# nyu-systems/Grendel-GS

Measured on NVIDIA H100. Metric: train-step Gaussians/s (preprocess+forward+loss+backward), higher is better.
Workload: dtype f32

## Files before the change

grendel-gs_b200/csrc/loss.cu:

```cuda
#include "common.cuh"

#define LS_TILE 32
#define LS_HALO 5
#define LS_IN (LS_TILE + 2 * LS_HALO)
#define LS_THREADS 256

__device__ __constant__ float c_gauss[11];
static unsigned long long g_gauss_ready = 0ull;

static int ensure_gauss() {
    int dev = 0;
    GS_CUDA_TRY(cudaGetDevice(&dev));
    if (dev < 64 && ((g_gauss_ready >> dev) & 1ull)) return GS_OK;
    float g[11], s = 0.f;
    for (int k = 0; k < 11; k++) { g[k] = (float)exp(-((double)(k - 5) * (k - 5)) / (2.0 * 1.5 * 1.5)); s += g[k]; }
    for (int k = 0; k < 11; k++) g[k] = g[k] / s;
    GS_CUDA_TRY(cudaMemcpyToSymbol(c_gauss, g, sizeof(g)));
    if (dev < 64) g_gauss_ready |= 1ull << dev;
    return GS_OK;
}

extern "C" size_t gs_loss_temp_bytes(int rows, int image_width) {
    return (size_t)9 * (size_t)(rows > 0 ? rows : 0) * (size_t)image_width * sizeof(float) + 256;
}

struct LossViews {
    int row0[GS_MAX_VIEWS], rows[GS_MAX_VIEWS];
    int crow0[GS_MAX_VIEWS], crow1[GS_MAX_VIEWS];
    const uint8_t *gt[GS_MAX_VIEWS];
    unsigned long long map_off[GS_MAX_VIEWS];
};

__global__ void __launch_bounds__(LS_THREADS)
k_loss_fwd(int W, int H, const LossViews lv, const float *__restrict__ image, float *__restrict__ maps,
           double *__restrict__ sums) {
    __shared__ float s_x[LS_IN][LS_IN + 1], s_y[LS_IN][LS_IN + 1];
    __shared__ float s_h[5][LS_IN][LS_TILE + 1];
    __shared__ float s_red[2][LS_THREADS / 32];
    const int view = blockIdx.z;
    const int row0 = lv.row0[view], rows = lv.rows[view], crow0 = lv.crow0[view], crow1 = lv.crow1[view];
    const int tx0 = blockIdx.x * LS_TILE, ty0 = blockIdx.y * LS_TILE;
    if (ty0 >= rows) return;
    const size_t HW = (size_t)H * W, SW = (size_t)rows * W;
    const uint8_t *__restrict__ gt = lv.gt[view];
    image += (size_t)view * 3 * HW;
    maps += lv.map_off[view];
    sums += 2 * view;
    const float C1 = 0.01f * 0.01f, C2 = 0.03f * 0.03f;
    float l1 = 0.f, ss = 0.f;
    for (int ch = 0; ch < 3; ch++) {
        for (int k = threadIdx.x; k < LS_IN * LS_IN; k += LS_THREADS) {
            const int r = k / LS_IN, c = k % LS_IN;
            const int y = ty0 + r - LS_HALO, x = tx0 + c - LS_HALO;
            float vx = 0.f, vy = 0.f;
            if (y >= 0 && y < rows && x >= 0 && x < W) {
                vx = image[ch * HW + (size_t)(row0 + y) * W + x];
                vy = fminf(1.f, fmaxf(0.f, (float)gt[ch * SW + (size_t)y * W + x] / 255.0f));
            }
            s_x[r][c] = vx; s_y[r][c] = vy;
        }
        __syncthreads();
        for (int k = threadIdx.x; k < LS_IN * (LS_TILE / 4); k += LS_THREADS) {
            const int r = k / (LS_TILE / 4), c0 = (k % (LS_TILE / 4)) * 4;
            float wx[14], wy[14];
#pragma unroll
            for (int t = 0; t < 14; t++) { wx[t] = s_x[r][c0 + t]; wy[t] = s_y[r][c0 + t]; }
#pragma unroll
            for (int q = 0; q < 4; q++) {
                float a0 = 0.f, a1 = 0.f, a2 = 0.f, a3 = 0.f, a4 = 0.f;
#pragma unroll
                for (int t = 0; t < 11; t++) {
                    const float g = c_gauss[t], vx = wx[q + t], vy = wy[q + t];
                    a0 += g * vx; a1 += g * vy; a2 += g * vx * vx; a3 += g * vy * vy; a4 += g * vx * vy;
                }
                s_h[0][r][c0 + q] = a0; s_h[1][r][c0 + q] = a1; s_h[2][r][c0 + q] = a2; s_h[3][r][c0 + q] = a3;
                s_h[4][r][c0 + q] = a4;
            }
        }
        __syncthreads();
        {
            const int c = threadIdx.x % LS_TILE, r0 = (threadIdx.x / LS_TILE) * 4, x = tx0 + c;
            float m1[4] = {0.f, 0.f, 0.f, 0.f}, m2[4] = {0.f, 0.f, 0.f, 0.f}, e11[4] = {0.f, 0.f, 0.f, 0.f},
                  e22[4] = {0.f, 0.f, 0.f, 0.f}, e12[4] = {0.f, 0.f, 0.f, 0.f};
#pragma unroll
            for (int t = 0; t < 14; t++) {
                const float v0 = s_h[0][r0 + t][c], v1 = s_h[1][r0 + t][c], v2 = s_h[2][r0 + t][c], v3 = s_h[3][r0 + t][c],
                            v4 = s_h[4][r0 + t][c];
#pragma unroll
                for (int q = 0; q < 4; q++) {
                    if (t - q >= 0 && t - q < 11) {
                        const float g = c_gauss[t - q];
                        m1[q] += g * v0; m2[q] += g * v1; e11[q] += g * v2; e22[q] += g * v3; e12[q] += g * v4;
                    }
                }
            }
#pragma unroll
            for (int q = 0; q < 4; q++) {
                const int r = r0 + q, y = ty0 + r;
                if (y < rows && x < W) {
                    const size_t o = (size_t)ch * SW + (size_t)y * W + x;
                    if (y < crow0 || y >= crow1) {
                        maps[o] = 0.f; maps[3 * SW + o] = 0.f; maps[6 * SW + o] = 0.f;
                    } else {
                        const float s1 = e11[q] - m1[q] * m1[q], s2 = e22[q] - m2[q] * m2[q], s12 = e12[q] - m1[q] * m2[q];
                        const float A = 2.f * m1[q] * m2[q] + C1, B = 2.f * s12 + C2,
                                    Cc = m1[q] * m1[q] + m2[q] * m2[q] + C1, D = s1 + s2 + C2;
                        const float iCD = 1.f / (Cc * D);
                        ss += A * B * iCD;
                        const float vx = s_x[r + LS_HALO][c + LS_HALO], vy = s_y[r + LS_HALO][c + LS_HALO];
                        l1 += fabsf(vx - vy);
                        maps[o] = 2.f * m2[q] * (B - A) * iCD - 2.f * m1[q] * A * B * (D - Cc) * iCD * iCD;
                        maps[3 * SW + o] = -A * B * iCD / D;
                        maps[6 * SW + o] = 2.f * A * iCD;
                    }
                }
            }
        }
        __syncthreads();
    }
#pragma unroll
    for (int o = 16; o > 0; o >>= 1) { l1 += __shfl_xor_sync(0xffffffffu, l1, o); ss += __shfl_xor_sync(0xffffffffu, ss, o); }
    if ((threadIdx.x & 31) == 0) { s_red[0][threadIdx.x >> 5] = l1; s_red[1][threadIdx.x >> 5] = ss; }
    __syncthreads();
    if (threadIdx.x == 0) {
        double a = 0.0, b = 0.0;
        for (int w = 0; w < LS_THREADS / 32; w++) { a += (double)s_red[0][w]; b += (double)s_red[1][w]; }
        atomicAdd(&sums[0], a); atomicAdd(&sums[1], b);
    }
}

__global__ void k_loss_finalize(int n, const double *__restrict__ sums, double inv_norm, float *__restrict__ out) {
    const int k = blockIdx.x * blockDim.x + threadIdx.x;
    if (k < 2 * n) out[k] = (float)(sums[k] * inv_norm);
}

__global__ void __launch_bounds__(LS_THREADS)
k_loss_bwd(int W, int H, const LossViews lv, const float *__restrict__ image, const float *__restrict__ maps,
           const float *__restrict__ grad_l1, const float *__restrict__ grad_ssim, float inv_norm,
           float *__restrict__ dimg) {
    __shared__ float s_m[3][LS_IN][LS_IN + 1];
    __shared__ float s_h[3][LS_IN][LS_TILE + 1];
    const int view = blockIdx.z;
    const int row0 = lv.row0[view], rows = lv.rows[view], crow0 = lv.crow0[view], crow1 = lv.crow1[view];
    const int tx0 = blockIdx.x * LS_TILE, ty0 = blockIdx.y * LS_TILE;
    if (ty0 >= rows) return;
    const size_t HW = (size_t)H * W, SW = (size_t)rows * W;
    const uint8_t *__restrict__ gt = lv.gt[view];
    image += (size_t)view * 3 * HW;
    dimg += (size_t)view * 3 * HW;
    maps += lv.map_off[view];
    const float gl1 = grad_l1[view] * inv_norm, gss = grad_ssim[view] * inv_norm;
    for (int ch = 0; ch < 3; ch++) {
        for (int k = threadIdx.x; k < LS_IN * LS_IN; k += LS_THREADS) {
            const int r = k / LS_IN, c = k % LS_IN;
            const int y = ty0 + r - LS_HALO, x = tx0 + c - LS_HALO;
            float v0 = 0.f, v1 = 0.f, v2 = 0.f;
            if (y >= 0 && y < rows && x >= 0 && x < W) {
                const size_t o = (size_t)ch * SW + (size_t)y * W + x;
                v0 = maps[o]; v1 = maps[3 * SW + o]; v2 = maps[6 * SW + o];
            }
            s_m[0][r][c] = v0; s_m[1][r][c] = v1; s_m[2][r][c] = v2;
        }
        __syncthreads();
        for (int k = threadIdx.x; k < LS_IN * (LS_TILE / 4); k += LS_THREADS) {
            const int r = k / (LS_TILE / 4), c0 = (k % (LS_TILE / 4)) * 4;
            float w0[14], w1[14], w2[14];
#pragma unroll
            for (int t = 0; t < 14; t++) { w0[t] = s_m[0][r][c0 + t]; w1[t] = s_m[1][r][c0 + t]; w2[t] = s_m[2][r][c0 + t]; }
#pragma unroll
            for (int q = 0; q < 4; q++) {
                float a0 = 0.f, a1 = 0.f, a2 = 0.f;
#pragma unroll
                for (int t = 0; t < 11; t++) {
                    const float g = c_gauss[t];
                    a0 += g * w0[q + t]; a1 += g * w1[q + t]; a2 += g * w2[q + t];
                }
                s_h[0][r][c0 + q] = a0; s_h[1][r][c0 + q] = a1; s_h[2][r][c0 + q] = a2;
            }
        }
        __syncthreads();
        {
            const int c = threadIdx.x % LS_TILE, r0 = (threadIdx.x / LS_TILE) * 4, x = tx0 + c;
            float b0[4] = {0.f, 0.f, 0.f, 0.f}, b1[4] = {0.f, 0.f, 0.f, 0.f}, b2[4] = {0.f, 0.f, 0.f, 0.f};
#pragma unroll
            for (int t = 0; t < 14; t++) {
                const float v0 = s_h[0][r0 + t][c], v1 = s_h[1][r0 + t][c], v2 = s_h[2][r0 + t][c];
#pragma unroll
                for (int q = 0; q < 4; q++) {
                    if (t - q >= 0 && t - q < 11) {
                        const float g = c_gauss[t - q];
                        b0[q] += g * v0; b1[q] += g * v1; b2[q] += g * v2;
                    }
                }
            }
#pragma unroll
            for (int q = 0; q < 4; q++) {
                const int y = ty0 + r0 + q;
                if (y < rows && x < W) {
                    const size_t oi = ch * HW + (size_t)(row0 + y) * W + x;
                    const float vx = image[oi];
                    const float vy = fminf(1.f, fmaxf(0.f, (float)gt[ch * SW + (size_t)y * W + x] / 255.0f));
                    const float d = vx - vy;
                    const float sgn = (y < crow0 || y >= crow1) ? 0.f : (d > 0.f ? 1.f : (d < 0.f ? -1.f : 0.f));
                    dimg[oi] = gl1 * sgn + gss * (b0[q] + 2.f * vx * b1[q] + vy * b2[q]);
                }
            }
        }
        __syncthreads();
    }
}

#define LS_HEADER_1 ((size_t)256)
#define LS_HEADER_B ((size_t)(2 * sizeof(double) * GS_MAX_VIEWS))

static int make_loss_views(int num_views, int H, int W, const int32_t *rows4, const void *const *gts, LossViews &lv,
                           int *max_rows, size_t *sum_rows) {
    GS_REQUIRE(num_views >= 1 && num_views <= GS_MAX_VIEWS, "num_views must be in [1, GS_MAX_VIEWS]");
    GS_REQUIRE(H > 0 && W > 0 && rows4 && gts, "sizes");
    size_t off = 0;
    int mx = 0;
    for (int v = 0; v < GS_MAX_VIEWS; v++) {
        lv.row0[v] = lv.rows[v] = lv.crow0[v] = lv.crow1[v] = 0;
        lv.gt[v] = nullptr;
        lv.map_off[v] = 0ull;
        if (v >= num_views) continue;
        const int row0 = rows4[4 * v], row1 = rows4[4 * v + 1], c0 = rows4[4 * v + 2], c1 = rows4[4 * v + 3];
        const int rows = row1 - row0;
        GS_REQUIRE(row0 >= 0 && row1 <= H && rows >= 0, "strip rows");
        if (rows == 0) continue;
        GS_REQUIRE(c0 >= row0 && c1 <= row1 && c1 >= c0, "count rows must lie inside [row0,row1)");
        GS_REQUIRE(gts[v] != nullptr, "null ground-truth pointer");
        lv.row0[v] = row0; lv.rows[v] = rows; lv.crow0[v] = c0 - row0; lv.crow1[v] = c1 - row0;
        lv.gt[v] = (const uint8_t *)gts[v];
        lv.map_off[v] = (unsigned long long)off;
        off += (size_t)9 * rows * W;
        mx = rows > mx ? rows : mx;
    }
    *max_rows = mx;
    *sum_rows = off / ((size_t)9 * W);
    return GS_OK;
}

static int loss_forward_impl(int num_views, int H, int W, const int32_t *rows4, const float *image, const void *const *gts,
                             float *out, void *temp, size_t temp_bytes, size_t header, cudaStream_t stream) {
    GS_REQUIRE(image && out && temp, "null pointer");
    LossViews lv;
    int max_rows = 0;
    size_t sum_rows = 0;
    int rc = make_loss_views(num_views, H, W, rows4, gts, lv, &max_rows, &sum_rows);
    if (rc != GS_OK) return rc;
    if (temp_bytes < header + (size_t)9 * sum_rows * W * sizeof(float)) {
        gs_set_error("gs_loss_forward: temp too small");
        return GS_ENOMEM;
    }
    rc = ensure_gauss();
    if (rc != GS_OK) return rc;
    double *sums = (double *)temp;
    float *maps = (float *)((char *)temp + header);
    GS_CUDA_TRY(cudaMemsetAsync(sums, 0, 2 * sizeof(double) * (size_t)num_views, stream));
    GsStageTimer timer(GS_STAGE_LOSS_FWD, stream);
    if (max_rows > 0) {
        dim3 grid((W + LS_TILE - 1) / LS_TILE, (max_rows + LS_TILE - 1) / LS_TILE, num_views);
        k_loss_fwd<<<grid, LS_THREADS, 0, stream>>>(W, H, lv, image, maps, sums);
        GS_LAUNCH_CHECK();
    }
    k_loss_finalize<<<1, 2 * GS_MAX_VIEWS, 0, stream>>>(num_views, sums, 1.0 / (3.0 * (double)H * (double)W), out);
    GS_LAUNCH_CHECK();
    return GS_OK;
}

static int loss_backward_impl(int num_views, int H, int W, const int32_t *rows4, const float *image,
                              const void *const *gts, const void *temp, const float *grad_l1, const float *grad_ssim,
                              float *dimg, size_t header, cudaStream_t stream) {
    GS_REQUIRE(image && temp && grad_l1 && grad_ssim && dimg, "null pointer");
    LossViews lv;
    int max_rows = 0;
    size_t sum_rows = 0;
    int rc = make_loss_views(num_views, H, W, rows4, gts, lv, &max_rows, &sum_rows);
    if (rc != GS_OK) return rc;
    rc = ensure_gauss();
    if (rc != GS_OK) return rc;
    const float *maps = (const float *)((const char *)temp + header);
    const size_t HW = (size_t)H * W;
    if (num_views == 1) {
        const int row0 = lv.row0[0], row1 = lv.row0[0] + lv.rows[0];
        for (int ch = 0; ch < 3; ch++) {
            if (row0 > 0) GS_CUDA_TRY(cudaMemsetAsync(dimg + ch * HW, 0, sizeof(float) * (size_t)row0 * W, stream));
            if (row1 < H)
                GS_CUDA_TRY(cudaMemsetAsync(dimg + ch * HW + (size_t)row1 * W, 0, sizeof(float) * (size_t)(H - row1) * W, stream));
        }
    } else if (sum_rows < (size_t)num_views * H) {
        GS_CUDA_TRY(cudaMemsetAsync(dimg, 0, sizeof(float) * 3 * HW * (size_t)num_views, stream));
    }
    if (max_rows == 0) return GS_OK;
    dim3 grid((W + LS_TILE - 1) / LS_TILE, (max_rows + LS_TILE - 1) / LS_TILE, num_views);
    GsStageTimer timer(GS_STAGE_LOSS_BWD, stream);
    k_loss_bwd<<<grid, LS_THREADS, 0, stream>>>(W, H, lv, image, maps, grad_l1, grad_ssim,
                                                (float)(1.0 / (3.0 * (double)H * (double)W)), dimg);
    GS_LAUNCH_CHECK();
    return GS_OK;
}

extern "C" int gs_loss_forward(int image_height, int image_width, int row0, int row1, int count_row0, int count_row1,
                               const float *image, const uint8_t *gt_u8, float *out_l1_ssim, void *temp,
                               size_t temp_bytes, void *stream_) {
    GS_REQUIRE(row1 > row0, "strip rows");
    GS_REQUIRE(gt_u8, "null pointer");
    const int32_t rows4[4] = {row0, row1, count_row0, count_row1};
    const void *gts[1] = {gt_u8};
    return loss_forward_impl(1, image_height, image_width, rows4, image, gts, out_l1_ssim, temp, temp_bytes, LS_HEADER_1,
                             (cudaStream_t)stream_);
}

extern "C" size_t gs_loss_temp_bytes_batched(int num_views, const int32_t *rows4_host, int image_width) {
    size_t rows = 0;
    for (int v = 0; v < num_views && rows4_host; v++) {
        const int r = rows4_host[4 * v + 1] - rows4_host[4 * v];
        rows += r > 0 ? (size_t)r : 0;
    }
    return LS_HEADER_B + (size_t)9 * rows * (size_t)(image_width > 0 ? image_width : 0) * sizeof(float) + 256;
}

extern "C" int gs_loss_forward_batched(int num_views, int image_height, int image_width, const int32_t *rows4_host,
                                       const float *image, const void *const *gt_u8_ptrs_host, float *out_l1_ssim,
                                       void *temp, size_t temp_bytes, void *stream_) {
    return loss_forward_impl(num_views, image_height, image_width, rows4_host, image, gt_u8_ptrs_host, out_l1_ssim, temp,
                             temp_bytes, LS_HEADER_B, (cudaStream_t)stream_);
}

extern "C" int gs_loss_backward(int image_height, int image_width, int row0, int row1, int count_row0, int count_row1,
                                const float *image, const uint8_t *gt_u8, const void *temp, const float *grad_l1,
                                const float *grad_ssim, float *dL_dimage, void *stream_) {
    GS_REQUIRE(row1 > row0, "strip rows");
    GS_REQUIRE(gt_u8, "null pointer");
    const int32_t rows4[4] = {row0, row1, count_row0, count_row1};
    const void *gts[1] = {gt_u8};
    return loss_backward_impl(1, image_height, image_width, rows4, image, gts, temp, grad_l1, grad_ssim, dL_dimage,
                              LS_HEADER_1, (cudaStream_t)stream_);
}

extern "C" int gs_loss_backward_batched(int num_views, int image_height, int image_width, const int32_t *rows4_host,
                                        const float *image, const void *const *gt_u8_ptrs_host, const void *temp,
                                        const float *grad_l1, const float *grad_ssim, float *dL_dimage, void *stream_) {
    return loss_backward_impl(num_views, image_height, image_width, rows4_host, image, gt_u8_ptrs_host, temp, grad_l1,
                              grad_ssim, dL_dimage, LS_HEADER_B, (cudaStream_t)stream_);
}
```

Measured before the change: 596.6 million.

## Restructure SSIM loss kernels to load rows directly with vector loads into wider tiles

The forward and backward SSIM/L1 loss kernels drop the shared-memory staging of raw inputs. The horizontal Gaussian pass now reads image, ground-truth and map rows straight from global memory, using float4 and packed-byte loads when alignment allows. Tiles widen to 64x32 and each thread in the vertical pass computes 8 rows, with launch-bound occupancy hints and a max-shared carveout. The L1 term moves into the horizontal pass, and the uint8-to-float conversion is replaced by an exactly rounded reciprocal multiply. The intent is to cut shared-memory traffic and halo overhead, at the cost of more registers and possible spills under the occupancy bounds.

New measurement: 611.8 million (median of 6 runs). 1.03x the previous value.

```diff
diff --git a/grendel-gs_b200/csrc/loss.cu b/grendel-gs_b200/csrc/loss.cu
--- a/grendel-gs_b200/csrc/loss.cu
+++ b/grendel-gs_b200/csrc/loss.cu
@@ -1,23 +1,65 @@
 #include "common.cuh"
 
-#define LS_TILE 32
+#define LS_TW 64
+#define LS_TH 32
 #define LS_HALO 5
-#define LS_IN (LS_TILE + 2 * LS_HALO)
+#define LS_WR (LS_TH + 2 * LS_HALO)
 #define LS_THREADS 256
+#define LS_Q 4
+#define LS_ROW_ITEMS (LS_WR * LS_TW / LS_Q)
+#define LS_R 8
+#define LS_FWD_SMEM ((size_t)5 * LS_WR * LS_TW * sizeof(float))
+static_assert(LS_TW * LS_TH / LS_R == LS_THREADS, "the column pass covers the tile in one round");
+static_assert(LS_TW % 4 == 0, "16-byte loads start on a multiple of 4 columns");
 
 __device__ __constant__ float c_gauss[11];
-static unsigned long long g_gauss_ready = 0ull;
-
-static int ensure_gauss() {
-    int dev = 0;
-    GS_CUDA_TRY(cudaGetDevice(&dev));
-    if (dev < 64 && ((g_gauss_ready >> dev) & 1ull)) return GS_OK;
-    float g[11], s = 0.f;
-    for (int k = 0; k < 11; k++) { g[k] = (float)exp(-((double)(k - 5) * (k - 5)) / (2.0 * 1.5 * 1.5)); s += g[k]; }
-    for (int k = 0; k < 11; k++) g[k] = g[k] / s;
-    GS_CUDA_TRY(cudaMemcpyToSymbol(c_gauss, g, sizeof(g)));
-    if (dev < 64) g_gauss_ready |= 1ull << dev;
-    return GS_OK;
+static unsigned long long g_loss_ready = 0ull;
+
+
+__device__ __forceinline__ float gt_unit(unsigned u) {
+    const float f = (float)u, r = 1.0f / 255.0f;
+    const float q = __fmul_rn(f, r);
+    return __fmaf_rn(__fmaf_rn(-q, 255.0f, f), r, q);
+}
+
+__device__ __forceinline__ void load14(const float *__restrict__ row, int gx0, int W, bool vec, float v[14]) {
+    if (vec) {
+        float f[20];
+#pragma unroll
+        for (int j = 0; j < 5; j++) {
+            const int gx = gx0 - 3 + 4 * j;
+            float4 q = make_float4(0.f, 0.f, 0.f, 0.f);
+            if (gx >= 0 && gx < W) q = __ldg(reinterpret_cast<const float4 *>(row + gx));
+            f[4 * j] = q.x; f[4 * j + 1] = q.y; f[4 * j + 2] = q.z; f[4 * j + 3] = q.w;
+        }
+#pragma unroll
+        for (int t = 0; t < 14; t++) v[t] = f[t + 3];
+    } else {
+#pragma unroll
+        for (int t = 0; t < 14; t++) {
+            const int gx = gx0 + t;
+            v[t] = (gx >= 0 && gx < W) ? __ldg(row + gx) : 0.f;
+        }
+    }
+}
+
+__device__ __forceinline__ void load14_gt(const uint8_t *__restrict__ row, int gx0, int W, bool vec, float v[14]) {
+    if (vec) {
+        unsigned w[5];
+#pragma unroll
+        for (int j = 0; j < 5; j++) {
+            const int gx = gx0 - 3 + 4 * j;
+            w[j] = (gx >= 0 && gx < W) ? __ldg(reinterpret_cast<const unsigned *>(row + gx)) : 0u;
+        }
+#pragma unroll
+        for (int t = 0; t < 14; t++) v[t] = gt_unit((w[(t + 3) >> 2] >> (8 * ((t + 3) & 3))) & 0xffu);
+    } else {
+#pragma unroll
+        for (int t = 0; t < 14; t++) {
+            const int gx = gx0 + t;
+            v[t] = (gx >= 0 && gx < W) ? gt_unit(__ldg(row + gx)) : 0.f;
+        }
+    }
 }
 
 extern "C" size_t gs_loss_temp_bytes(int rows, int image_width) {
@@ -31,72 +73,81 @@
     unsigned long long map_off[GS_MAX_VIEWS];
 };
 
-__global__ void __launch_bounds__(LS_THREADS)
-k_loss_fwd(int W, int H, const LossViews lv, const float *__restrict__ image, float *__restrict__ maps,
+__global__ void __launch_bounds__(LS_THREADS, 4)
+k_loss_fwd(int W, int H, const LossViews lv, int vec, const float *__restrict__ image, float *__restrict__ maps,
            double *__restrict__ sums) {
-    __shared__ float s_x[LS_IN][LS_IN + 1], s_y[LS_IN][LS_IN + 1];
-    __shared__ float s_h[5][LS_IN][LS_TILE + 1];
+    extern __shared__ __align__(16) float s_dyn[];
+    float(*s_h)[LS_WR][LS_TW] = reinterpret_cast<float(*)[LS_WR][LS_TW]>(s_dyn);
     __shared__ float s_red[2][LS_THREADS / 32];
     const int view = blockIdx.z;
     const int row0 = lv.row0[view], rows = lv.rows[view], crow0 = lv.crow0[view], crow1 = lv.crow1[view];
-    const int tx0 = blockIdx.x * LS_TILE, ty0 = blockIdx.y * LS_TILE;
+    const int tx0 = blockIdx.x * LS_TW, ty0 = blockIdx.y * LS_TH;
     if (ty0 >= rows) return;
     const size_t HW = (size_t)H * W, SW = (size_t)rows * W;
     const uint8_t *__restrict__ gt = lv.gt[view];
-    image += (size_t)view * 3 * HW;
+    image += (size_t)view * 3 * HW + (size_t)row0 * W;
     maps += lv.map_off[view];
     sums += 2 * view;
     const float C1 = 0.01f * 0.01f, C2 = 0.03f * 0.03f;
+    const int c = threadIdx.x % LS_TW, r0 = (threadIdx.x / LS_TW) * LS_R, x = tx0 + c;
     float l1 = 0.f, ss = 0.f;
     for (int ch = 0; ch < 3; ch++) {
-        for (int k = threadIdx.x; k < LS_IN * LS_IN; k += LS_THREADS) {
-            const int r = k / LS_IN, c = k % LS_IN;
-            const int y = ty0 + r - LS_HALO, x = tx0 + c - LS_HALO;
-            float vx = 0.f, vy = 0.f;
-            if (y >= 0 && y < rows && x >= 0 && x < W) {
-                vx = image[ch * HW + (size_t)(row0 + y) * W + x];
-                vy = fminf(1.f, fmaxf(0.f, (float)gt[ch * SW + (size_t)y * W + x] / 255.0f));
-            }
-            s_x[r][c] = vx; s_y[r][c] = vy;
-        }
-        __syncthreads();
-        for (int k = threadIdx.x; k < LS_IN * (LS_TILE / 4); k += LS_THREADS) {
-            const int r = k / (LS_TILE / 4), c0 = (k % (LS_TILE / 4)) * 4;
-            float wx[14], wy[14];
-#pragma unroll
-            for (int t = 0; t < 14; t++) { wx[t] = s_x[r][c0 + t]; wy[t] = s_y[r][c0 + t]; }
-#pragma unroll
-            for (int q = 0; q < 4; q++) {
-                float a0 = 0.f, a1 = 0.f, a2 = 0.f, a3 = 0.f, a4 = 0.f;
-#pragma unroll
-                for (int t = 0; t < 11; t++) {
-                    const float g = c_gauss[t], vx = wx[q + t], vy = wy[q + t];
-                    a0 += g * vx; a1 += g * vy; a2 += g * vx * vx; a3 += g * vy * vy; a4 += g * vx * vy;
-                }
-                s_h[0][r][c0 + q] = a0; s_h[1][r][c0 + q] = a1; s_h[2][r][c0 + q] = a2; s_h[3][r][c0 + q] = a3;
-                s_h[4][r][c0 + q] = a4;
-            }
+        for (int k = threadIdx.x; k < LS_ROW_ITEMS; k += LS_THREADS) {
+            const int r = k / (LS_TW / LS_Q), c0 = (k % (LS_TW / LS_Q)) * LS_Q;
+            const int y = ty0 + r - LS_HALO, gx0 = tx0 + c0 - LS_HALO;
+            float a[5][LS_Q];
+#pragma unroll
+            for (int m = 0; m < 5; m++)
+#pragma unroll
+                for (int q = 0; q < LS_Q; q++) a[m][q] = 0.f;
+            if (y >= 0 && y < rows) {
+                float wx[LS_Q + 10], wy[LS_Q + 10];
+                load14(image + ch * HW + (size_t)y * W, gx0, W, vec, wx);
+                load14_gt(gt + ch * SW + (size_t)y * W, gx0, W, vec, wy);
+                if (r >= LS_HALO && r < LS_HALO + LS_TH && y >= crow0 && y < crow1) {
+#pragma unroll
+                    for (int q = 0; q < LS_Q; q++)
+                        if (tx0 + c0 + q < W) l1 += fabsf(wx[q + LS_HALO] - wy[q + LS_HALO]);
+                }
+#pragma unroll
+                for (int t = 0; t < LS_Q + 10; t++) {
+                    const float vx = wx[t], vy = wy[t], xx = vx * vx, yy = vy * vy, xy = vx * vy;
+#pragma unroll
+                    for (int q = 0; q < LS_Q; q++) {
+                        if (t - q >= 0 && t - q < 11) {
+                            const float g = c_gauss[t - q];
+                            a[0][q] = fmaf(g, vx, a[0][q]); a[1][q] = fmaf(g, vy, a[1][q]);
+                            a[2][q] = fmaf(g, xx, a[2][q]); a[3][q] = fmaf(g, yy, a[3][q]);
+                            a[4][q] = fmaf(g, xy, a[4][q]);
+                        }
+                    }
+                }
+            }
+#pragma unroll
+            for (int m = 0; m < 5; m++)
+                *reinterpret_cast<float4 *>(&s_h[m][r][c0]) = make_float4(a[m][0], a[m][1], a[m][2], a[m][3]);
         }
         __syncthreads();
         {
-            const int c = threadIdx.x % LS_TILE, r0 = (threadIdx.x / LS_TILE) * 4, x = tx0 + c;
-            float m1[4] = {0.f, 0.f, 0.f, 0.f}, m2[4] = {0.f, 0.f, 0.f, 0.f}, e11[4] = {0.f, 0.f, 0.f, 0.f},
-                  e22[4] = {0.f, 0.f, 0.f, 0.f}, e12[4] = {0.f, 0.f, 0.f, 0.f};
-#pragma unroll
-            for (int t = 0; t < 14; t++) {
-                const float v0 = s_h[0][r0 + t][c], v1 = s_h[1][r0 + t][c], v2 = s_h[2][r0 + t][c], v3 = s_h[3][r0 + t][c],
-                            v4 = s_h[4][r0 + t][c];
-#pragma unroll
-                for (int q = 0; q < 4; q++) {
+            float m1[LS_R], m2[LS_R], e11[LS_R], e22[LS_R], e12[LS_R];
+#pragma unroll
+            for (int q = 0; q < LS_R; q++) m1[q] = m2[q] = e11[q] = e22[q] = e12[q] = 0.f;
+#pragma unroll
+            for (int t = 0; t < LS_R + 10; t++) {
+                const float v0 = s_h[0][r0 + t][c], v1 = s_h[1][r0 + t][c], v2 = s_h[2][r0 + t][c],
+                            v3 = s_h[3][r0 + t][c], v4 = s_h[4][r0 + t][c];
+#pragma unroll
+                for (int q = 0; q < LS_R; q++) {
                     if (t - q >= 0 && t - q < 11) {
                         const float g = c_gauss[t - q];
-                        m1[q] += g * v0; m2[q] += g * v1; e11[q] += g * v2; e22[q] += g * v3; e12[q] += g * v4;
+                        m1[q] = fmaf(g, v0, m1[q]); m2[q] = fmaf(g, v1, m2[q]); e11[q] = fmaf(g, v2, e11[q]);
+                        e22[q] = fmaf(g, v3, e22[q]); e12[q] = fmaf(g, v4, e12[q]);
                     }
                 }
             }
 #pragma unroll
-            for (int q = 0; q < 4; q++) {
-                const int r = r0 + q, y = ty0 + r;
+            for (int q = 0; q < LS_R; q++) {
+                const int y = ty0 + r0 + q;
                 if (y < rows && x < W) {
                     const size_t o = (size_t)ch * SW + (size_t)y * W + x;
                     if (y < crow0 || y >= crow1) {
@@ -107,8 +158,6 @@
                                     Cc = m1[q] * m1[q] + m2[q] * m2[q] + C1, D = s1 + s2 + C2;
                         const float iCD = 1.f / (Cc * D);
                         ss += A * B * iCD;
-                        const float vx = s_x[r + LS_HALO][c + LS_HALO], vy = s_y[r + LS_HALO][c + LS_HALO];
-                        l1 += fabsf(vx - vy);
                         maps[o] = 2.f * m2[q] * (B - A) * iCD - 2.f * m1[q] * A * B * (D - Cc) * iCD * iCD;
                         maps[3 * SW + o] = -A * B * iCD / D;
                         maps[6 * SW + o] = 2.f * A * iCD;
@@ -134,72 +183,70 @@
     if (k < 2 * n) out[k] = (float)(sums[k] * inv_norm);
 }
 
-__global__ void __launch_bounds__(LS_THREADS)
-k_loss_bwd(int W, int H, const LossViews lv, const float *__restrict__ image, const float *__restrict__ maps,
+__global__ void __launch_bounds__(LS_THREADS, 5)
+k_loss_bwd(int W, int H, const LossViews lv, int vec, const float *__restrict__ image, const float *__restrict__ maps,
            const float *__restrict__ grad_l1, const float *__restrict__ grad_ssim, float inv_norm,
            float *__restrict__ dimg) {
-    __shared__ float s_m[3][LS_IN][LS_IN + 1];
-    __shared__ float s_h[3][LS_IN][LS_TILE + 1];
+    __shared__ __align__(16) float s_h[3][LS_WR][LS_TW];
     const int view = blockIdx.z;
     const int row0 = lv.row0[view], rows = lv.rows[view], crow0 = lv.crow0[view], crow1 = lv.crow1[view];
-    const int tx0 = blockIdx.x * LS_TILE, ty0 = blockIdx.y * LS_TILE;
+    const int tx0 = blockIdx.x * LS_TW, ty0 = blockIdx.y * LS_TH;
     if (ty0 >= rows) return;
     const size_t HW = (size_t)H * W, SW = (size_t)rows * W;
     const uint8_t *__restrict__ gt = lv.gt[view];
     image += (size_t)view * 3 * HW;
     dimg += (size_t)view * 3 * HW;
     maps += lv.map_off[view];
-    const float gl1 = grad_l1[view] * inv_norm, gss = grad_ssim[view] * inv_norm;
+    const int c = threadIdx.x % LS_TW, r0 = (threadIdx.x / LS_TW) * LS_R, x = tx0 + c;
     for (int ch = 0; ch < 3; ch++) {
-        for (int k = threadIdx.x; k < LS_IN * LS_IN; k += LS_THREADS) {
-            const int r = k / LS_IN, c = k % LS_IN;
-            const int y = ty0 + r - LS_HALO, x = tx0 + c - LS_HALO;
-            float v0 = 0.f, v1 = 0.f, v2 = 0.f;
-            if (y >= 0 && y < rows && x >= 0 && x < W) {
-                const size_t o = (size_t)ch * SW + (size_t)y * W + x;
-                v0 = maps[o]; v1 = maps[3 * SW + o]; v2 = maps[6 * SW + o];
-            }
-            s_m[0][r][c] = v0; s_m[1][r][c] = v1; s_m[2][r][c] = v2;
-        }
-        __syncthreads();
-        for (int k = threadIdx.x; k < LS_IN * (LS_TILE / 4); k += LS_THREADS) {
-            const int r = k / (LS_TILE / 4), c0 = (k % (LS_TILE / 4)) * 4;
-            float w0[14], w1[14], w2[14];
-#pragma unroll
-            for (int t = 0; t < 14; t++) { w0[t] = s_m[0][r][c0 + t]; w1[t] = s_m[1][r][c0 + t]; w2[t] = s_m[2][r][c0 + t]; }
-#pragma unroll
-            for (int q = 0; q < 4; q++) {
-                float a0 = 0.f, a1 = 0.f, a2 = 0.f;
-#pragma unroll
-                for (int t = 0; t < 11; t++) {
-                    const float g = c_gauss[t];
-                    a0 += g * w0[q + t]; a1 += g * w1[q + t]; a2 += g * w2[q + t];
-                }
-                s_h[0][r][c0 + q] = a0; s_h[1][r][c0 + q] = a1; s_h[2][r][c0 + q] = a2;
-            }
+        for (int k = threadIdx.x; k < LS_ROW_ITEMS; k += LS_THREADS) {
+            const int r = k / (LS_TW / LS_Q), c0 = (k % (LS_TW / LS_Q)) * LS_Q;
+            const int y = ty0 + r - LS_HALO, gx0 = tx0 + c0 - LS_HALO;
+            float a[3][LS_Q];
+#pragma unroll
+            for (int m = 0; m < 3; m++)
+#pragma unroll
+                for (int q = 0; q < LS_Q; q++) a[m][q] = 0.f;
+            if (y >= 0 && y < rows) {
+#pragma unroll
+                for (int m = 0; m < 3; m++) {
+                    float w[LS_Q + 10];
+                    load14(maps + (size_t)(3 * m + ch) * SW + (size_t)y * W, gx0, W, vec, w);
+#pragma unroll
+                    for (int t = 0; t < LS_Q + 10; t++)
+#pragma unroll
+                        for (int q = 0; q < LS_Q; q++)
+                            if (t - q >= 0 && t - q < 11) a[m][q] = fmaf(c_gauss[t - q], w[t], a[m][q]);
+                }
+            }
+#pragma unroll
+            for (int m = 0; m < 3; m++)
+                *reinterpret_cast<float4 *>(&s_h[m][r][c0]) = make_float4(a[m][0], a[m][1], a[m][2], a[m][3]);
         }
         __syncthreads();
         {
-            const int c = threadIdx.x % LS_TILE, r0 = (threadIdx.x / LS_TILE) * 4, x = tx0 + c;
-            float b0[4] = {0.f, 0.f, 0.f, 0.f}, b1[4] = {0.f, 0.f, 0.f, 0.f}, b2[4] = {0.f, 0.f, 0.f, 0.f};
-#pragma unroll
-            for (int t = 0; t < 14; t++) {
+            float b0[LS_R], b1[LS_R], b2[LS_R];
+#pragma unroll
+            for (int q = 0; q < LS_R; q++) b0[q] = b1[q] = b2[q] = 0.f;
+#pragma unroll
+            for (int t = 0; t < LS_R + 10; t++) {
                 const float v0 = s_h[0][r0 + t][c], v1 = s_h[1][r0 + t][c], v2 = s_h[2][r0 + t][c];
 #pragma unroll
-                for (int q = 0; q < 4; q++) {
+                for (int q = 0; q < LS_R; q++) {
                     if (t - q >= 0 && t - q < 11) {
                         const float g = c_gauss[t - q];
-                        b0[q] += g * v0; b1[q] += g * v1; b2[q] += g * v2;
+                        b0[q] = fmaf(g, v0, b0[q]); b1[q] = fmaf(g, v1, b1[q]); b2[q] = fmaf(g, v2, b2[q]);
                     }
                 }
             }
-#pragma unroll
-            for (int q = 0; q < 4; q++) {
+            const float gl1 = grad_l1[view] * inv_norm, gss = grad_ssim[view] * inv_norm;
+#pragma unroll
+            for (int q = 0; q < LS_R; q++) {
                 const int y = ty0 + r0 + q;
                 if (y < rows && x < W) {
                     const size_t oi = ch * HW + (size_t)(row0 + y) * W + x;
                     const float vx = image[oi];
-                    const float vy = fminf(1.f, fmaxf(0.f, (float)gt[ch * SW + (size_t)y * W + x] / 255.0f));
+                    const float vy = gt_unit(gt[ch * SW + (size_t)y * W + x]);
                     const float d = vx - vy;
                     const float sgn = (y < crow0 || y >= crow1) ? 0.f : (d > 0.f ? 1.f : (d < 0.f ? -1.f : 0.f));
                     dimg[oi] = gl1 * sgn + gss * (b0[q] + 2.f * vx * b1[q] + vy * b2[q]);
@@ -208,6 +255,23 @@
         }
         __syncthreads();
     }
+}
+
+static bool aligned(const void *p, size_t n) { return ((uintptr_t)p & (n - 1)) == 0; }
+
+static int ensure_loss_setup() {
+    int dev = 0;
+    GS_CUDA_TRY(cudaGetDevice(&dev));
+    if (dev < 64 && ((g_loss_ready >> dev) & 1ull)) return GS_OK;
+    float g[11], s = 0.f;
+    for (int k = 0; k < 11; k++) { g[k] = (float)exp(-((double)(k - 5) * (k - 5)) / (2.0 * 1.5 * 1.5)); s += g[k]; }
+    for (int k = 0; k < 11; k++) g[k] = g[k] / s;
+    GS_CUDA_TRY(cudaMemcpyToSymbol(c_gauss, g, sizeof(g)));
+    GS_CUDA_TRY(cudaFuncSetAttribute(k_loss_fwd, cudaFuncAttributeMaxDynamicSharedMemorySize, (int)LS_FWD_SMEM));
+    GS_CUDA_TRY(cudaFuncSetAttribute(k_loss_fwd, cudaFuncAttributePreferredSharedMemoryCarveout, cudaSharedmemCarveoutMaxShared));
+    GS_CUDA_TRY(cudaFuncSetAttribute(k_loss_bwd, cudaFuncAttributePreferredSharedMemoryCarveout, cudaSharedmemCarveoutMaxShared));
+    if (dev < 64) g_loss_ready |= 1ull << dev;
+    return GS_OK;
 }
 
 #define LS_HEADER_1 ((size_t)256)
@@ -253,15 +317,17 @@
         gs_set_error("gs_loss_forward: temp too small");
         return GS_ENOMEM;
     }
-    rc = ensure_gauss();
+    rc = ensure_loss_setup();
     if (rc != GS_OK) return rc;
     double *sums = (double *)temp;
     float *maps = (float *)((char *)temp + header);
     GS_CUDA_TRY(cudaMemsetAsync(sums, 0, 2 * sizeof(double) * (size_t)num_views, stream));
     GsStageTimer timer(GS_STAGE_LOSS_FWD, stream);
     if (max_rows > 0) {
-        dim3 grid((W + LS_TILE - 1) / LS_TILE, (max_rows + LS_TILE - 1) / LS_TILE, num_views);
-        k_loss_fwd<<<grid, LS_THREADS, 0, stream>>>(W, H, lv, image, maps, sums);
+        bool vec = W % 4 == 0 && aligned(image, 16);
+        for (int v = 0; v < num_views; v++) vec = vec && aligned(lv.gt[v], 4);
+        dim3 grid((W + LS_TW - 1) / LS_TW, (max_rows + LS_TH - 1) / LS_TH, num_views);
+        k_loss_fwd<<<grid, LS_THREADS, LS_FWD_SMEM, stream>>>(W, H, lv, vec ? 1 : 0, image, maps, sums);
         GS_LAUNCH_CHECK();
     }
     k_loss_finalize<<<1, 2 * GS_MAX_VIEWS, 0, stream>>>(num_views, sums, 1.0 / (3.0 * (double)H * (double)W), out);
@@ -278,7 +344,7 @@
     size_t sum_rows = 0;
     int rc = make_loss_views(num_views, H, W, rows4, gts, lv, &max_rows, &sum_rows);
     if (rc != GS_OK) return rc;
-    rc = ensure_gauss();
+    rc = ensure_loss_setup();
     if (rc != GS_OK) return rc;
     const float *maps = (const float *)((const char *)temp + header);
     const size_t HW = (size_t)H * W;
@@ -293,9 +359,10 @@
         GS_CUDA_TRY(cudaMemsetAsync(dimg, 0, sizeof(float) * 3 * HW * (size_t)num_views, stream));
     }
     if (max_rows == 0) return GS_OK;
-    dim3 grid((W + LS_TILE - 1) / LS_TILE, (max_rows + LS_TILE - 1) / LS_TILE, num_views);
+    const bool vec = W % 4 == 0 && aligned(maps, 16);
+    dim3 grid((W + LS_TW - 1) / LS_TW, (max_rows + LS_TH - 1) / LS_TH, num_views);
     GsStageTimer timer(GS_STAGE_LOSS_BWD, stream);
-    k_loss_bwd<<<grid, LS_THREADS, 0, stream>>>(W, H, lv, image, maps, grad_l1, grad_ssim,
+    k_loss_bwd<<<grid, LS_THREADS, 0, stream>>>(W, H, lv, vec ? 1 : 0, image, maps, grad_l1, grad_ssim,
                                                 (float)(1.0 / (3.0 * (double)H * (double)W)), dimg);
     GS_LAUNCH_CHECK();
     return GS_OK;
diff --git a/profiles/loss_timing.py b/profiles/loss_timing.py
--- /dev/null
+++ b/profiles/loss_timing.py
@@ -0,0 +1,123 @@
+#!/usr/bin/env python
+import argparse
+import json
+import os
+import subprocess
+import sys
+
+ROOT = os.path.dirname(os.path.dirname(os.path.abspath(__file__)))
+for _p in (ROOT, os.path.join(ROOT, "grendel-gs_b200")):
+    if _p not in sys.path:
+        sys.path.insert(0, _p)
+
+CASES = [("1080p x1", 1080, 1920, 1), ("1080p x4", 1080, 1920, 4), ("2160p x1", 2160, 3840, 1)]
+FWD_BYTES_PER_PX, BWD_BYTES_PER_PX = 51, 63
+
+
+def card():
+    import torch
+    name = torch.cuda.get_device_name(0)
+    try:
+        q = subprocess.run(["nvidia-smi", "--id=0", "--query-gpu=power.limit,clocks.max.sm", "--format=csv,noheader"],
+                           capture_output=True, text=True, timeout=30).stdout.strip().splitlines()[0]
+    except (OSError, subprocess.SubprocessError, IndexError):
+        q = "unknown"
+    return name, q
+
+
+def time_case(H, W, B, iters):
+    import ctypes as C
+    import torch
+    from gs_b200 import _lib
+    dev = torch.device("cuda", 0)
+    g = torch.Generator(device=dev).manual_seed(H + B)
+    images = torch.rand((B, 3, H, W), device=dev, generator=g) * 1.1 - 0.05
+    gts = [torch.randint(0, 256, (3, H, W), device=dev, generator=g, dtype=torch.uint8) for _ in range(B)]
+    rows4 = (C.c_int32 * (4 * B))(*[v for _ in range(B) for v in (0, H, 0, H)])
+    gptrs = (C.c_void_p * B)(*[t.data_ptr() for t in gts])
+    tb = _lib.query("gs_loss_temp_bytes_batched", B, rows4, W)
+    temp = torch.empty((tb,), dtype=torch.uint8, device=dev)
+    out = torch.empty((B, 2), device=dev)
+    gl1 = torch.full((B,), 0.8, device=dev)
+    gss = torch.full((B,), -0.2, device=dev)
+    dimg = torch.empty_like(images)
+    s = torch.cuda.current_stream().cuda_stream
+
+    def fwd():
+        _lib.call("gs_loss_forward_batched", B, H, W, rows4, images.data_ptr(), gptrs, out.data_ptr(), temp.data_ptr(),
+                  tb, s)
+
+    def bwd():
+        _lib.call("gs_loss_backward_batched", B, H, W, rows4, images.data_ptr(), gptrs, temp.data_ptr(), gl1.data_ptr(),
+                  gss.data_ptr(), dimg.data_ptr(), s)
+
+    res = {}
+    for name, fn in (("fwd", fwd), ("bwd", bwd)):
+        for _ in range(20):
+            fn()
+        torch.cuda.synchronize()
+        a, b = torch.cuda.Event(enable_timing=True), torch.cuda.Event(enable_timing=True)
+        a.record()
+        for _ in range(iters):
+            fn()
+        b.record()
+        b.synchronize()
+        res[name] = a.elapsed_time(b) / iters
+    px = B * H * W
+    return dict(fwd_ms=round(res["fwd"], 4), bwd_ms=round(res["bwd"], 4), sum_ms=round(res["fwd"] + res["bwd"], 4),
+                fwd_GBps=round(FWD_BYTES_PER_PX * px / res["fwd"] / 1e6, 1),
+                bwd_GBps=round(BWD_BYTES_PER_PX * px / res["bwd"] / 1e6, 1),
+                loss=[round(float(v), 7) for v in out.reshape(-1).tolist()[:2]])
+
+
+def worker(iters):
+    import torch
+    if not torch.cuda.is_available():
+        sys.exit("loss_timing.py needs a GPU")
+    for label, H, W, B in CASES:
+        print(json.dumps(dict(case=label, **time_case(H, W, B, iters))), flush=True)
+        torch.cuda.empty_cache()
+
+
+def main():
+    ap = argparse.ArgumentParser()
+    ap.add_argument("--iters", type=int, default=300)
+    ap.add_argument("--rounds", type=int, default=3)
+    ap.add_argument("--ab", metavar="OTHER_LIB", default=None, help="a second build of libgrendel_gs_b200.so to alternate with")
+    ap.add_argument("--worker", action="store_true", help=argparse.SUPPRESS)
+    args = ap.parse_args()
+    if args.worker:
+        worker(args.iters)
+        return
+    import torch
+    if not torch.cuda.is_available():
+        sys.exit("loss_timing.py needs a GPU")
+    name, limit = card()
+    print(json.dumps(dict(gpu=name, power_limit_and_max_sm_clock=limit, iters=args.iters,
+                          fwd_bytes_per_px=FWD_BYTES_PER_PX, bwd_bytes_per_px=BWD_BYTES_PER_PX)), flush=True)
+    libs = {"this tree": os.environ.get("GS_B200_LIB") or os.path.join(ROOT, "grendel-gs_b200", "lib",
+                                                                        "libgrendel_gs_b200.so")}
+    if args.ab:
+        libs["other"] = os.path.abspath(args.ab)
+    results = {k: {} for k in libs}
+    for rnd in range(args.rounds if args.ab else 1):
+        for key, path in libs.items():
+            env = dict(os.environ, GS_B200_LIB=path)
+            r = subprocess.run([sys.executable, os.path.abspath(__file__), "--worker", "--iters", str(args.iters)],
+                               env=env, capture_output=True, text=True, timeout=900)
+            if r.returncode != 0:
+                sys.exit(f"{key} ({path}) failed:\n{r.stderr[-3000:]}")
+            for line in r.stdout.strip().splitlines():
+                d = json.loads(line)
+                print(json.dumps(dict(lib=key, round=rnd, **d)), flush=True)
+                results[key].setdefault(d["case"], []).append(d)
+    med = lambda v: sorted(v)[len(v) // 2]
+    summary = {}
+    for key, cases in results.items():
+        summary[key] = {c: {f: med([d[f] for d in ds]) for f in ("fwd_ms", "bwd_ms", "sum_ms", "fwd_GBps", "bwd_GBps")}
+                        for c, ds in cases.items()}
+    print(json.dumps(dict(summary=summary)), flush=True)
+
+
+if __name__ == "__main__":
+    main()
```
